# ZackAttack614/BlackBird

Measured on AMD Instinct MI355X. Metric: selfplay_games_per_sec, higher is better.
Workload: dtype f32 (float32 operands split exactly into 3 bf16 values, 6 bf16 MFMA products each, f32 accumulate)

## Files before the change

blackbird_amd/csrc/tree.hip.h:

```cpp
#pragma once
#include "games.hip.h"
#include "rng.hip.h"
#include "starts.h"
#include "stamps.hip.h"

#define NODE_EXPANDED 1
#define NODE_TERMINAL 2
#define NODE_CACHED 4
#define LEAF_RECORDED 0x40000000
#define CHILD_NONE (-1)
#define CHILD_TERM_BIT 0x40000000

template <class G>
struct alignas(128) DenseNode {
    int32_t flags;
    uint32_t legal_mask;
    int32_t all;
    int32_t serial;
    double sq;
    double pad0;
    int32_t N[G::S];
    float Q[G::S];
    int32_t child[G::S];
    alignas(128) double cP[G::S];
    float W[G::S];
    typename G::State st;
};

struct ExampleHdr {
    uint32_t game_id;
    uint16_t ply;
    uint8_t player;
    int8_t z;
    uint32_t total;
    uint32_t n_children;
};

#define BB_SLOTS_TREE(B, Q, R)                                                                     \
    B(int32_t, root, 1) B(int32_t, root_N, 1) B(int32_t, n_nodes, 1) B(int32_t, ply, 1) B(int32_t, sims_left, 1)           \
    B(int32_t, pend_leaf, 1) B(int32_t, pend_expand, 1) B(int32_t, path_len, 1)                                            \
    B(int32_t, game_lid, 1)                                             \
    B(int32_t, sim_serial, 1) B(float, root_W, 1)                                                                          \
    B(int8_t, root_pp, 1)                                   \
    B(uint32_t, path, MP)                                                                \
        \
    R(int32_t, path_N, MP) R(int32_t, path_all, MP)       \
    R(float, path_W, MP)                                                               \
    Q(int32_t, leaf_flags, 1)
#define BB_SLOTS_ANC(X)                                                                                 \
       \
    X(uint32_t, anc, ANC)                                                                                                   \
    X(int32_t, anc_len, 1) X(int32_t, top_N, 1)
#define BB_SLOTS_MAILBOX(B, Q)                                                 \
    B(uint32_t, leaf_game_id, 1) B(int32_t, leaf_serial, 1) B(float, eval_value, 1) Q(float, eval_policy, PS)              \
    B(uint64_t, evals, 1)                                                              \
    B(uint64_t, ctr, 8)
#define BB_SLOTS_OUT(X)                                                       \
    X(int32_t, out_action, 1) X(int32_t, out_root_plays, 1) X(int32_t, out_child_plays, S)                                 \
    X(float, out_root_winrate, 1) X(float, out_child_value, S)
#define BB_SLOTS_RESUME(X) X(int32_t, resume_cur, 1) X(int32_t, resume_depth, 1)
#define BB_SLOTS_POST(X) X(int, post_slot, 1)
#define BB_ROW_NONE(...)
#define BB_SLOT_ARRAYS(X) BB_SLOTS_TREE(X, X, X) BB_SLOTS_ANC(X) BB_SLOTS_MAILBOX(X, X) BB_SLOTS_OUT(X) BB_SLOTS_RESUME(X) BB_SLOTS_POST(X)
#define BB_SLOT_SHADOWED(X) BB_SLOTS_TREE(X, BB_ROW_NONE, BB_ROW_NONE) BB_SLOTS_MAILBOX(X, BB_ROW_NONE)
#define BB_SLOT_POINTER(T, f, per) T *f;
#define BB_SHADOW_MEMBER(T, f, per) T f[GW * (per)];
#define BB_SHADOW_LOAD(o, f, per) for (int i = threadIdx.x; i < n * (per); i += nthreads) f[i] = o.f[(size_t)g0 * (per) + i];
#define BB_SHADOW_STORE(o, f, per) for (int i = threadIdx.x; i < n * (per); i += nthreads) o.f[(size_t)g0 * (per) + i] = f[i];

struct TreeDev {
    int n_slots, node_cap, sims_per_move, max_plies, kind, max_depth, evaluator, priors_ones;
    int salt_per_game, max_games;
    int gpw;
    double c_puct;
    uint64_t seed, salt;
    uint32_t first_game_id;
    BB_SLOTS_TREE(BB_SLOT_POINTER, BB_SLOT_POINTER, BB_SLOT_POINTER)
    int track_anc;
    BB_SLOTS_ANC(BB_SLOT_POINTER)
    void *leaf_state;
    BB_SLOTS_MAILBOX(BB_SLOT_POINTER, BB_SLOT_POINTER)
    void *nodes;
    int n_games_target;
    double temp;
    uint8_t *examples;
    int32_t *game_hdr;
    int example_bytes;
    BB_SLOTS_OUT(BB_SLOT_POINTER)
    const double *in_u;
    BB_SLOTS_RESUME(BB_SLOT_POINTER)
    int *post_count;
    BB_SLOTS_POST(BB_SLOT_POINTER)
    int level_budget;
    int slot_offset;
    int lid_stride;
    int pool_g0;
    int *visit_pool;
    float noise_alpha;
    void *eval_cache;
    int eval_cache_log2;
    unsigned long long *eval_cache_ctr;
    unsigned long long *stamps;
    const void *starts;
    int n_starts;
    double temp_late;
    int temp_plies;
};

template <int STEP>
__device__ __forceinline__ int dpp_step_i(int v) {
    if (STEP == 0) return __builtin_amdgcn_update_dpp(v, v, 0xB1, 0xf, 0xf, false);
    if (STEP == 1) return __builtin_amdgcn_update_dpp(v, v, 0x4E, 0xf, 0xf, false);
    if (STEP == 2) return __builtin_amdgcn_update_dpp(v, v, 0x141, 0xf, 0xf, false);
    return __builtin_amdgcn_update_dpp(v, v, 0x140, 0xf, 0xf, false);
}
template <int STEP>
__device__ __forceinline__ double dpp_step_d(double v) {
    long long b = __double_as_longlong(v);
    int lo = dpp_step_i<STEP>((int)(b & 0xffffffffll)), hi = dpp_step_i<STEP>((int)(b >> 32));
    return __longlong_as_double(((long long)hi << 32) | (unsigned int)lo);
}

template <int S>
__device__ __forceinline__ int grp_sum_i(int v) {
    v += dpp_step_i<0>(v);
    v += dpp_step_i<1>(v);
    v += dpp_step_i<2>(v);
    if (S == 16) v += dpp_step_i<3>(v);
    return v;
}

template <int A, int S>
__device__ __forceinline__ double grp_np_sum(double x) {
    double a[A];
#pragma unroll
    for (int k = 0; k < A; k++) a[k] = __shfl(x, k, S);
    if (A < 8) {
        double res = 0.;
#pragma unroll
        for (int k = 0; k < A; k++) res += a[k];
        return res;
    } else {
        double r[8];
#pragma unroll
        for (int j = 0; j < 8; j++) r[j] = a[j];
        int i = 8;
        for (; i < A - (A % 8); i += 8)
            for (int j = 0; j < 8; j++) r[j] += a[i + j];
        double res = ((r[0] + r[1]) + (r[2] + r[3])) + ((r[4] + r[5]) + (r[6] + r[7]));
        for (; i < A; i++) res += a[i];
        return res;
    }
}

template <int S, int STEP>
__device__ __forceinline__ void argmax_step(double &u, int &idx, int &payload) {
    double ou = dpp_step_d<STEP>(u);
    int oi = dpp_step_i<STEP>(idx), op = dpp_step_i<STEP>(payload);
    if (ou > u || (ou == u && oi < idx)) {
        u = ou;
        idx = oi;
        payload = op;
    }
}
template <int S>
__device__ __forceinline__ int grp_argmax(double u, int idx, int &payload) {
    (void)idx;
    double m = u;
    m = __builtin_fmax(m, dpp_step_d<0>(m));
    m = __builtin_fmax(m, dpp_step_d<1>(m));
    m = __builtin_fmax(m, dpp_step_d<2>(m));
    if (S == 16) m = __builtin_fmax(m, dpp_step_d<3>(m));
    const unsigned long long eq = __ballot(u == m);
    const int l64 = (int)__lane_id();
    const unsigned grp = (unsigned)(eq >> (l64 & ~(S - 1))) & ((1u << S) - 1u);
    const int win = __ffs(grp) - 1;
    payload = __shfl(payload, win, S);
    return win;
}

__device__ __forceinline__ double puct_score(double q, double cPi, double sq, int Ni, bool legal) {
    double u = q + __ddiv_rn(cPi * sq, 1.0 + (double)Ni);
    return legal ? u : -1.0;
}
#ifndef BB_PUCT_FILTER
#define BB_PUCT_FILTER 1
#endif
template <int S>
__device__ __forceinline__ int grp_argmax_puct(float qf, double cPi, double sq, int Ni, bool legal, int &payload) {
#if BB_PUCT_FILTER
    const float num = (float)(cPi * sq);
    const float uf = legal ? __builtin_fmaf(num, __builtin_amdgcn_rcpf((float)(Ni + 1)), qf) : -1.0f;
    float mf = uf;
    mf = __builtin_fmaxf(mf, __int_as_float(dpp_step_i<0>(__float_as_int(mf))));
    mf = __builtin_fmaxf(mf, __int_as_float(dpp_step_i<1>(__float_as_int(mf))));
    mf = __builtin_fmaxf(mf, __int_as_float(dpp_step_i<2>(__float_as_int(mf))));
    if (S == 16) mf = __builtin_fmaxf(mf, __int_as_float(dpp_step_i<3>(__float_as_int(mf))));
    const bool mine = uf >= mf - mf * 0x1p-18f && uf >= 0.0f;
    const unsigned long long cand = __ballot(mine);
    const int l64 = (int)__lane_id();
    const unsigned grp = (unsigned)(cand >> (l64 & ~(S - 1))) & ((1u << S) - 1u);
    if (__ballot((grp & (grp - 1u)) != 0u || grp == 0u) == 0ull) {
        const int win = __ffs(grp) - 1;
        int p = mine ? payload : 0;
        p |= dpp_step_i<0>(p);
        p |= dpp_step_i<1>(p);
        p |= dpp_step_i<2>(p);
        if (S == 16) p |= dpp_step_i<3>(p);
        payload = p;
        return win;
    }
#endif
    return grp_argmax<S>(puct_score((double)qf, cPi, sq, Ni, legal), 0, payload);
}
__device__ __forceinline__ double child_q(const TreeDev &d, float Qi, float Wi, int Ni) {
    if (d.evaluator != 2) return (double)Qi;
    return Ni > 0 ? (double)Wi / (double)Ni : 0.0;
}

__device__ __forceinline__ uint32_t path_word(int node, int player, int a) {
    return ((uint32_t)node << 6) | ((uint32_t)player << 4) | (uint32_t)a;
}
#define ANC_BROKEN (-1)

template <class G, bool REC = false>
__device__ __forceinline__ void backup_path(const TreeDev &d, int g, int lane, DenseNode<G> *pool, int plen, float v01,
                                            int prev) {
    constexpr int S = G::S;
    const float vflip = 1.0f - v01;
    const size_t p0 = (size_t)g * G::MAXPATH;
    auto edge = [&](uint32_t e, int k) __attribute__((always_inline)) {
        const int a = e & 15, pl = (e >> 4) & 3;
        DenseNode<G> *pn = pool + (e >> 6);
        int n, all;
        float w;
        if constexpr (REC) { n = d.path_N[p0 + k]; all = d.path_all[p0 + k]; w = d.path_W[p0 + k]; }
        else { n = pn->N[a]; all = pn->all; w = pn->W[a]; }
        n += 1;
        all += 1;
        w += (pl == prev) ? v01 : vflip;
        pn->N[a] = n;
        pn->W[a] = w;
        pn->Q[a] = __fdiv_rn(w, (float)n);
        pn->all = all;
        pn->sq = __dsqrt_rn(1.0 + (double)all);
    };
    for (int k = lane; k < plen; k += S) edge(d.path[p0 + k], k);
    if constexpr (!REC) {
        if (d.track_anc) {
            const uint32_t *anc = d.anc + (size_t)g * (d.max_plies + 2);
            const int na = d.anc_len[g];
            for (int k = lane; k < na; k += S) edge(anc[k], 0);
            if (lane == 0) d.top_N[g] += 1;
        }
    }
    if (lane == 0) {
        d.root_N[g] += 1;
        int pp = d.root_pp[g];
        if (pp) d.root_W[g] += (pp == prev) ? v01 : vflip;
    }
}

template <class G, bool REC = false>
__device__ __forceinline__ void phase_apply(const TreeDev &d, int g, int lane) {
    using Node = DenseNode<G>;
    constexpr int S = G::S, A = G::A;
    const int leaf = d.pend_leaf[g];
    if (leaf < 0) return;
    int lf = 0;
    if constexpr (REC) lf = d.leaf_flags[g] & ~LEAF_RECORDED;
    Node *pool = (Node *)d.nodes + (size_t)(g + d.pool_g0) * d.node_cap;
    Node *node = pool + leaf;
    auto add_flag = [&](int bit) __attribute__((always_inline)) {
        if constexpr (REC) node->flags = lf | bit;
        else node->flags |= bit;
    };
    const typename G::State st = ((const typename G::State *)d.leaf_state)[g];
    const float v = d.eval_value[g];
    const int expand_rec = REC ? d.pend_expand[g] : 0;
    auto expand = [&]() __attribute__((always_inline)) { return REC ? expand_rec : d.pend_expand[g]; };
    if (expand()) {
        const uint32_t mask = G::legal_mask(st);
        double x = 0.0;
        if (lane < A) x = (double)d.eval_policy[(size_t)g * S + lane] * (double)((mask >> lane) & 1u);
        const double tot = grp_np_sum<A, S>(x);
        node->N[lane] = 0;
        node->Q[lane] = 0.f;
        node->W[lane] = 0.f;
        node->child[lane] = CHILD_NONE;
        node->cP[lane] = (lane < A) ? d.c_puct * __ddiv_rn(x, tot) : 0.0;
        if (lane == 0) {
            add_flag(NODE_EXPANDED);
            node->legal_mask = mask;
            node->all = 0;
            node->sq = 1.0;
        }
    }
    const int player = gs_player(st), prev = gs_prev(st);
    const bool f32_eval = REC || d.evaluator != 2;
    float v01 = v;
    if (f32_eval) {
        v01 = (v + 1.0f) * 0.5f;
        if (player != prev) v01 = 1.0f - v01;
    }
    if (f32_eval && !expand() && ((REC ? lf : node->flags) & NODE_TERMINAL) && lane == 0) {
        node->pad0 = (double)v01;
        add_flag(NODE_CACHED);
    }
    backup_path<G, REC>(d, g, lane, pool, d.path_len[g], v01, prev);
    if (lane == 0) d.pend_leaf[g] = -1;
}

template <class G>
__device__ __forceinline__ int create_child(const TreeDev &d, int g, DenseNode<G> *pool, DenseNode<G> *parent,
                                            const typename G::State &pst, int a, int lane, int &nn,
                                            typename G::State &st2, bool &terminal, int *flags_out = nullptr) {
    int idx = nn;
    st2 = pst;
    G::apply(st2, a);
    int w = G::winner(st2, a);
    terminal = w >= 0;
    if (idx >= d.node_cap) return CHILD_NONE;
    int word = idx | (terminal ? CHILD_TERM_BIT : 0);
    nn = idx + 1;
    const int cflags = (terminal ? (NODE_TERMINAL | ((w + 1) << 8)) : 0) | (gs_player(st2) << 4);
    if (flags_out) *flags_out = cflags;
    if (lane == 0) {
        DenseNode<G> *c = pool + idx;
        c->st = st2;
        c->flags = cflags;
        c->legal_mask = 0;
        c->all = 0;
        c->serial = idx;
        parent->child[a] = word;
        d.n_nodes[g] = idx + 1;
        d.ctr[(size_t)g * 8 + 2] += 1;
    }
    return word;
}

template <class G>
__device__ __forceinline__ uint32_t expand_ones(const TreeDev &d, DenseNode<G> *node, const typename G::State &st,
                                                int lane, double &cPi) {
    uint32_t mask = G::legal_mask(st);
    cPi = (lane < G::A && ((mask >> lane) & 1u)) ? d.c_puct * 1.0 : 0.0;
    node->N[lane] = 0;
    node->Q[lane] = 0.f;
    node->W[lane] = 0.f;
    node->child[lane] = CHILD_NONE;
    node->cP[lane] = cPi;
    if (lane == 0) {
        node->flags |= NODE_EXPANDED;
        node->legal_mask = mask;
        node->all = 0;
        node->sq = 1.0;
    }
    return mask;
}

template <class G>
__device__ __forceinline__ void post_leaf(const TreeDev &d, int g, int cur, const typename G::State &st, int flags_word, int expand,
                                          int depth) {
    ((typename G::State *)d.leaf_state)[g] = st;
    d.leaf_game_id[g] = d.first_game_id + (uint32_t)d.game_lid[g];
    d.leaf_serial[g] = cur;
    d.pend_leaf[g] = cur;
    if (d.leaf_flags) d.leaf_flags[g] = flags_word;
    d.pend_expand[g] = expand;
    d.path_len[g] = depth;
    d.sim_serial[g] += 1;
    d.evals[g] += 1;
}

template <class G>
__device__ void phase_select(const TreeDev &d, int g, int lane) {
    using Node = DenseNode<G>;
    constexpr int S = G::S, A = G::A;
    if (d.game_lid[g] < 0 || d.sims_left[g] <= 0) return;
    Node *pool = (Node *)d.nodes + (size_t)(g + d.pool_g0) * d.node_cap;
    uint32_t *path = d.path + (size_t)g * G::MAXPATH;
    int cur = d.root[g];
    int nn = d.n_nodes[g];
    int depth = 0, expand = 0, overflow = 0, term_leaf = 0;
    const bool inline_expand = d.priors_ones != 0;
    const bool fixed = d.kind == 1, rollout = d.evaluator == 2;
    typename G::State st;
    int flags = 0;
    bool have = false;
    IF_STAMPS(long long acc_load = 0, acc_iter = 0;)
    for (int it = 0;; it++) {
        IF_STAMPS(long long ts0 = clock64(); acc_iter++;)
        Node *node = pool + cur;
        typename G::State st_l = node->st;
        int flags_l = node->flags;
        uint32_t mask = node->legal_mask;
        double sq = node->sq;
        int Ni = node->N[lane];
        float Qi = node->Q[lane];
        float Wi = rollout ? node->W[lane] : 0.f;
        double cPi = node->cP[lane];
        int ci = node->child[lane];
        asm volatile("" ::"v"(flags_l), "v"(mask), "v"(sq), "v"(Ni), "v"(Qi), "v"(cPi), "v"(ci));
        IF_STAMPS(acc_load += clock64() - ts0;)
        if (!have) {
            st = st_l;
            flags = flags_l;
        }
        have = false;
        if (fixed && it >= d.max_depth) break;
        if (!(flags & NODE_EXPANDED)) {
            if (flags & NODE_TERMINAL) { term_leaf = 1; break; }
            if (!inline_expand) { expand = 1; break; }
            mask = expand_ones<G>(d, node, st, lane, cPi);
            if (!fixed) break;
            Ni = 0;
            Qi = 0.f;
            Wi = 0.f;
            sq = 1.0;
            ci = CHILD_NONE;
        }
        if (mask == 0) break;
        double u = puct_score(child_q(d, Qi, Wi, Ni), cPi, sq, Ni, lane < A && ((mask >> lane) & 1u));
        int child = ci;
        int a = grp_argmax<S>(u, lane, child);
        if (depth >= G::MAXPATH) { overflow = 1; break; }
        if (child == CHILD_NONE) {
            typename G::State st2;
            bool terminal;
            child = create_child<G>(d, g, pool, node, st, a, lane, nn, st2, terminal);
            if (child == CHILD_NONE) { overflow = 1; break; }
            if (lane == 0) path[depth] = path_word(cur, (flags >> 4) & 3, a);
            st = st2;
            flags = (terminal ? NODE_TERMINAL : 0) | (gs_player(st2) << 4);
            have = true;
        } else {
            if (lane == 0) path[depth] = path_word(cur, (flags >> 4) & 3, a);
        }
        depth++;
        cur = child & ~CHILD_TERM_BIT;
    }
    if (lane == 0) {
        IF_STAMPS(stamp_add(d.stamps, TS_ROW_LOAD, acc_load); stamp_add(d.stamps, TS_ITERATIONS, acc_iter); stamp_add(d.stamps, TS_DESCENTS, 1);)
        post_leaf<G>(d, g, cur, st, 0, expand, depth);
        d.sims_left[g] -= 1;
        uint64_t *c = d.ctr + (size_t)g * 8;
        c[0] += 1;
        c[1] += (uint64_t)depth;
        c[3] += (uint64_t)term_leaf;
        c[6] += (uint64_t)overflow;
    }
}

template <class G>
__global__ void __launch_bounds__(256) k_tree_step(TreeDev d) {
    constexpr int S = G::S;
    int t = blockIdx.x * blockDim.x + threadIdx.x;
    int wv = t >> 6, l64 = t & 63;
    if (l64 >= d.gpw * S) return;
    int g = wv * d.gpw + l64 / S, lane = l64 % S;
    if (g >= d.n_slots) return;
    const long long t0 = stamp_clock();
    phase_apply<G>(d, g, lane);
    const long long t1 = stamp_clock();
    __threadfence_block();
    const long long t2 = stamp_clock();
    phase_select<G>(d, g, lane);
    const long long t3 = stamp_clock();
    if ((threadIdx.x & 63) == 0) {
        stamp_add(d.stamps, TS_APPLY, t1 - t0);
        stamp_add(d.stamps, TS_FENCE, t2 - t1);
        stamp_add(d.stamps, TS_SELECT, t3 - t2);
        stamp_add(d.stamps, TS_WAVES, 1);
    }
}

template <class G>
__global__ void __launch_bounds__(256) k_tree_apply(TreeDev d) {
    constexpr int S = G::S;
    int t = blockIdx.x * blockDim.x + threadIdx.x;
    int g = t / S, lane = t % S;
    if (g >= d.n_slots) return;
    phase_apply<G>(d, g, lane);
}

template <class G>
__device__ __forceinline__ int choose_move(const TreeDev &d, int g, int lane, double temp, double u, int &total, int &Ni_out,
                           float &Wi_out) {
    using Node = DenseNode<G>;
    constexpr int S = G::S, A = G::A;
    Node *pool = (Node *)d.nodes + (size_t)(g + d.pool_g0) * d.node_cap;
    Node *node = pool + d.root[g];
    if (!(node->flags & NODE_EXPANDED)) {
        total = 0;
        Ni_out = 0;
        Wi_out = 0.f;
        return -3;
    }
    uint32_t mask = node->legal_mask;
    bool legal = lane < A && ((mask >> lane) & 1u);
    int Ni = legal ? node->N[lane] : 0;
    float Wi = legal ? node->W[lane] : 0.f;
    Ni_out = Ni;
    Wi_out = Wi;
    int all = grp_sum_i<S>(Ni);
    total = all;
    if (temp == 0.0) {
        double uu = puct_score(child_q(d, node->Q[lane], Wi, Ni), node->cP[lane], node->sq, Ni, legal);
        int dummy = 0;
        return grp_argmax<S>(uu, lane, dummy);
    }
    double it = 1.0 / temp;
    double w = (it == 1.0) ? (double)Ni : pow((double)Ni, it);
    double ws[A];
#pragma unroll
    for (int k = 0; k < A; k++) ws[k] = __shfl(w, k, S);
    double allp = 0.0;
#pragma unroll
    for (int k = 0; k < A; k++) allp += ws[k];
    if (!(allp > 0.0 && allp < INFINITY)) return -4;
    double last = 0.0;
#pragma unroll
    for (int k = 0; k < A; k++) last += __ddiv_rn(ws[k], allp);
    double run = 0.0;
    int act = A - 1;
    bool found = false;
#pragma unroll
    for (int k = 0; k < A; k++) {
        run += __ddiv_rn(ws[k], allp);
        if (!found && __ddiv_rn(run, last) > u) {
            act = k;
            found = true;
        }
    }
    return act;
}

template <class G>
__global__ void __launch_bounds__(256) k_sample(TreeDev d, double temp) {
    constexpr int S = G::S;
    int t = blockIdx.x * blockDim.x + threadIdx.x;
    int g = t / S, lane = t % S;
    if (g >= d.n_slots) return;
    if (d.game_lid[g] < 0) {
        if (lane == 0 && d.out_action) d.out_action[g] = -3;
        return;
    }
    double u = d.in_u ? d.in_u[g] : bb_u53(d.seed, d.first_game_id + (uint32_t)d.game_lid[g], (uint32_t)d.ply[g]);
    int total, Ni;
    float Wi;
    int act = choose_move<G>(d, g, lane, temp, u, total, Ni, Wi);
    if (d.out_child_plays) d.out_child_plays[(size_t)g * S + lane] = Ni;
    if (d.out_child_value) d.out_child_value[(size_t)g * S + lane] = Wi;
    if (lane == 0) {
        if (d.out_action) d.out_action[g] = act;
        if (d.out_root_plays) d.out_root_plays[g] = d.root_N[g];
        if (d.out_root_winrate) {
            int n = d.root_N[g];
            float w = d.root_W[g];
            d.out_root_winrate[g] = n > 0 ? ((d.evaluator == 2) ? (float)((double)w / (double)n) : __fdiv_rn(w, (float)n)) : 0.f;
        }
    }
}

template <class G, bool CHAIN = true>
__device__ __forceinline__ void advance_root(const TreeDev &d, int g, int lane, int a, typename G::State &new_st) {
    using Node = DenseNode<G>;
    Node *pool = (Node *)d.nodes + (size_t)(g + d.pool_g0) * d.node_cap;
    Node *node = pool + d.root[g];
    typename G::State st = node->st;
    if (!(node->flags & NODE_EXPANDED)) {
        new_st = st;
        G::apply(new_st, a);
        if (lane == 0) {
            Node *r = pool;
            r->st = new_st;
            r->flags = gs_player(new_st) << 4;
            r->serial = 0;
            d.n_nodes[g] = 1;
            d.root[g] = 0;
            d.root_N[g] = 0;
            d.root_W[g] = 0.f;
            d.root_pp[g] = 0;
            if (d.track_anc) {
                d.anc_len[g] = 0;
                d.top_N[g] = 0;
            }
        }
        return;
    }
    int child = node->child[a];
    int cn = node->N[a];
    float cw = node->W[a];
    if (child == CHILD_NONE) {
        bool terminal;
        int nn = d.n_nodes[g];
        child = create_child<G>(d, g, pool, node, st, a, lane, nn, new_st, terminal);
        if (child == CHILD_NONE) {
            child = 0;
            cn = 0;
            cw = 0.f;
            if (lane == 0) {
                pool->st = new_st;
                pool->flags = gs_player(new_st) << 4;
                d.n_nodes[g] = 1;
                d.ctr[(size_t)g * 8 + 6] += 1;
            }
        }
    } else {
        new_st = pool[child & ~CHILD_TERM_BIT].st;
    }
    if (lane == 0) {
        if (d.track_anc) {
            if (child == 0 && cn == 0 && d.n_nodes[g] == 1) {
                d.anc_len[g] = 0;
                d.top_N[g] = 0;
            } else if constexpr (!CHAIN) {
                if (d.anc_len[g] < d.max_plies + 2) {
                    d.anc[(size_t)g * (d.max_plies + 2) + d.anc_len[g]] = path_word(d.root[g], gs_player(st), a);
                    d.anc_len[g] += 1;
                }
            } else {
                const int na = d.anc_len[g], cap = d.max_plies + 2;
                if (na >= 0 && na < cap) {
                    d.anc[(size_t)g * cap + na] = path_word(d.root[g], gs_player(st), a);
                    d.anc_len[g] = na + 1;
                } else {
                    d.anc_len[g] = ANC_BROKEN;
                }
            }
        }
        d.root[g] = child & ~CHILD_TERM_BIT;
        d.root_N[g] = cn;
        d.root_W[g] = cw;
        d.root_pp[g] = (int8_t)gs_player(st);
    }
}

template <class G>
__global__ void __launch_bounds__(256) k_reset_roots(TreeDev d) {
    int g = blockIdx.x * blockDim.x + threadIdx.x;
    if (g >= d.n_slots || !d.track_anc || d.game_lid[g] < 0 || d.anc_len[g] <= 0) return;
    {
        const int na = d.anc_len[g];
        const bool parked = d.resume_cur[g] >= 0, posted = d.pend_leaf[g] >= 0;
        const int plen = parked ? d.resume_depth[g] : d.path_len[g];
        if (parked || posted) {
            if (plen + na <= G::MAXPATH) {
                uint32_t *path = d.path + (size_t)g * G::MAXPATH;
                const uint32_t *anc = d.anc + (size_t)g * (d.max_plies + 2);
                for (int k = plen - 1; k >= 0; k--) path[k + na] = path[k];
                for (int k = 0; k < na; k++) path[k] = anc[k];
                if (parked) d.resume_depth[g] = plen + na;
                else d.path_len[g] = plen + na;
            } else {
                d.ctr[(size_t)g * 8 + 6] += 1;
            }
        }
    }
    d.root[g] = (int)(d.anc[(size_t)g * (d.max_plies + 2)] >> 6);
    d.root_N[g] = d.top_N[g];
    d.root_W[g] = 0.f;
    d.root_pp[g] = 0;
    d.anc_len[g] = 0;
}

template <class G>
__global__ void __launch_bounds__(64) k_node_view(TreeDev d, int g, int node, int32_t *child_out, int32_t *plays_out, float *value_out,
                                                   typename G::State *state_out, int32_t *info_out) {
    using Node = DenseNode<G>;
    const int lane = threadIdx.x;
    if (lane >= G::S) return;
    Node *pool = (Node *)d.nodes + (size_t)(g + d.pool_g0) * d.node_cap;
    if (node < 0) node = d.root[g];
    const Node *n = pool + node;
    const bool exp = (n->flags & NODE_EXPANDED) != 0;
    child_out[lane] = exp ? n->child[lane] : CHILD_NONE;
    plays_out[lane] = exp ? n->N[lane] : 0;
    value_out[lane] = exp ? n->W[lane] : 0.f;
    if (lane == 0) {
        *state_out = n->st;
        info_out[0] = n->flags;
        info_out[1] = (int32_t)(exp ? n->legal_mask : 0u);
        info_out[2] = node;
    }
}

template <class G>
__global__ void __launch_bounds__(256) k_move_roots(TreeDev d, const int32_t *actions) {
    constexpr int S = G::S;
    int t = blockIdx.x * blockDim.x + threadIdx.x;
    int g = t / S, lane = t % S;
    if (g >= d.n_slots) return;
    int a = actions[g];
    if (a < 0 || a >= G::A || d.game_lid[g] < 0) return;
    typename G::State ns;
    advance_root<G>(d, g, lane, a, ns);
    if (lane == 0) d.ply[g] += 1;
}

template <class G>
__device__ __forceinline__ void reset_slot(const TreeDev &d, int g, int lid, const typename G::State &st) {
    using Node = DenseNode<G>;
    Node *pool = (Node *)d.nodes + (size_t)(g + d.pool_g0) * d.node_cap;
    pool->st = st;
    pool->flags = gs_player(st) << 4;
    pool->legal_mask = 0;
    pool->all = 0;
    pool->serial = 0;
    d.n_nodes[g] = 1;
    d.root[g] = 0;
    d.root_N[g] = 0;
    d.root_W[g] = 0.f;
    d.root_pp[g] = 0;
    d.ply[g] = 0;
    d.pend_leaf[g] = -1;
    d.pend_expand[g] = 0;
    d.path_len[g] = 0;
    d.sim_serial[g] = 0;
    d.game_lid[g] = lid;
    if (d.leaf_flags) d.leaf_flags[g] = 0;
    if (d.track_anc) {
        d.anc_len[g] = 0;
        d.top_N[g] = 0;
    }
}

template <class G>
__global__ void __launch_bounds__(256) k_set_roots(TreeDev d, int n, const int32_t *slots,
                                                   const typename G::State *states, const uint32_t *game_ids) {
    int i = blockIdx.x * blockDim.x + threadIdx.x;
    if (i >= n) return;
    int g = slots ? slots[i] : i;
    if (g < 0 || g >= d.n_slots) return;
    reset_slot<G>(d, g, game_ids ? (int)game_ids[i] : g, states[i]);
    d.sims_left[g] = 0;
}

__global__ void __launch_bounds__(256) k_add_sims(TreeDev d, int sims, const uint8_t *mask = nullptr) {
    int g = blockIdx.x * blockDim.x + threadIdx.x;
    if (g >= d.n_slots) return;
    if (d.game_lid[g] >= 0 && (!mask || mask[g])) d.sims_left[g] = sims;
}

template <class G>
__global__ void __launch_bounds__(256) k_get_roots(TreeDev d, typename G::State *out) {
    int g = blockIdx.x * blockDim.x + threadIdx.x;
    if (g >= d.n_slots) return;
    out[g] = ((DenseNode<G> *)d.nodes + (size_t)(g + d.pool_g0) * d.node_cap + d.root[g])->st;
}

template <class G>
__device__ __forceinline__ typename G::State start_state(const TreeDev &d, int lid) {
    const typename G::State *t = (const typename G::State *)d.starts;
    if (t && lid >= 0) return t[lid % d.n_starts];
    return G::initial();
}

template <class G>
__global__ void __launch_bounds__(256) k_check_starts(int n, const typename G::State *states, uint8_t *verdict) {
    int i = blockIdx.x * blockDim.x + threadIdx.x;
    if (i >= n) return;
    const typename G::State st = states[i];
    int v = BB_START_OK;
    if (G::winner(st, -1) >= 0) v = BB_START_FINISHED;
    else if (G::legal_mask(st) == 0) v = BB_START_NO_MOVE;
    verdict[i] = (uint8_t)v;
}

template <class G>
__global__ void __launch_bounds__(256) k_selfplay_begin(TreeDev d) {
    int g = blockIdx.x * blockDim.x + threadIdx.x;
    if (g >= d.n_slots) return;
    if (g + d.slot_offset < d.n_games_target) {
        reset_slot<G>(d, g, g + d.slot_offset, start_state<G>(d, g + d.slot_offset));
        d.sims_left[g] = d.sims_per_move;
    } else {
        reset_slot<G>(d, g, -1, start_state<G>(d, -1));
        d.sims_left[g] = 0;
    }
}

template <class G>
__device__ __forceinline__ uint8_t *example_ptr(const TreeDev &d, int lid, int ply) {
    return d.examples + ((size_t)lid * (d.max_plies + 1) + ply) * d.example_bytes;
}

template <class G>
__device__ __forceinline__ void write_example(const TreeDev &d, int lid, int ply, const typename G::State &st, int lane, int Ni,
                              int total, uint32_t gid) {
    uint8_t *p = example_ptr<G>(d, lid, ply);
    if (lane == 0) {
        ExampleHdr h;
        h.game_id = gid;
        h.ply = (uint16_t)ply;
        h.player = (uint8_t)gs_player(st);
        h.z = 0;
        h.total = (uint32_t)total;
        h.n_children = G::A;
        *(ExampleHdr *)p = h;
        *(typename G::State *)(p + sizeof(ExampleHdr)) = st;
    }
    ((uint32_t *)(p + sizeof(ExampleHdr) + sizeof(typename G::State)))[lane] = (uint32_t)Ni;
}

template <class G, bool CHAIN = true>
__device__ __forceinline__ void selfplay_move_body(const TreeDev &d, int g, int lane) {
    using Node = DenseNode<G>;
    constexpr int S = G::S;
    int lid = d.game_lid[g];
    if (lid < 0) return;
    Node *pool = (Node *)d.nodes + (size_t)(g + d.pool_g0) * d.node_cap;
    typename G::State st = pool[d.root[g]].st;
    uint32_t gid = d.first_game_id + (uint32_t)lid;
    int ply = d.ply[g];
    double u = bb_u53(d.seed, gid, (uint32_t)ply);
    int total, Ni;
    float Wi;
    int act = choose_move<G>(d, g, lane, ply < d.temp_plies ? d.temp : d.temp_late, u, total, Ni, Wi);
    if (act < 0) {
        if (lane == 0) {
            d.game_lid[g] = -1;
            d.ctr[(size_t)g * 8 + 6] += 1;
        }
        return;
    }
    write_example<G>(d, lid, ply, st, lane, Ni, total, gid);
    typename G::State ns;
    advance_root<G, CHAIN>(d, g, lane, act, ns);
    __threadfence_block();
    ply += 1;
    int w = G::winner(ns, -1);
    bool over = w >= 0 || ply >= d.max_plies;
    if (!over) {
        if (lane == 0) {
            d.ply[g] = ply;
            d.sims_left[g] = d.sims_per_move;
            d.ctr[(size_t)g * 8 + 5] += 1;
        }
        return;
    }
    write_example<G>(d, lid, ply, ns, lane, 0, 0, gid);
    __threadfence_block();
    for (int k = lane; k <= ply; k += S) {
        ExampleHdr *h = (ExampleHdr *)example_ptr<G>(d, lid, k);
        h->z = (w <= 0) ? 0 : (h->player == w ? 1 : -1);
    }
    __threadfence();
    if (lane == 0) {
        int32_t *gh = d.game_hdr + (size_t)lid * 4;
        gh[0] = ply + 1;
        gh[1] = w;
        gh[2] = ply;
        __threadfence();
        gh[3] = 1;
        uint64_t *c = d.ctr + (size_t)g * 8;
        c[4] += 1;
        c[5] += 1;
        c[7] += (uint64_t)(ply + 1);
        int next = lid + d.lid_stride;
        if (next < d.n_games_target) {
            reset_slot<G>(d, g, next, start_state<G>(d, next));
            d.sims_left[g] = d.sims_per_move;
        } else {
            d.game_lid[g] = -1;
            d.sims_left[g] = 0;
        }
    }
}

template <class G>
__global__ void __launch_bounds__(256) k_selfplay_move(TreeDev d) {
    constexpr int S = G::S;
    int t = blockIdx.x * blockDim.x + threadIdx.x;
    int g = t / S, lane = t % S;
    if (g >= d.n_slots) return;
    phase_apply<G>(d, g, lane);
    __threadfence_block();
    selfplay_move_body<G>(d, g, lane);
}

struct NoPostHook {
    __device__ __forceinline__ void operator()(int, int) const {}
};
template <class G, bool REC = false, class OnPost = NoPostHook>
__device__ bool async_game(const TreeDev &d, int g, int lane, OnPost on_post = OnPost(), LevelStamps *light_out = nullptr) {
    using Node = DenseNode<G>;
    constexpr int S = G::S, A = G::A;
    if (d.game_lid[g] < 0) return false;
    Node *pool = (Node *)d.nodes + (size_t)(g + d.pool_g0) * d.node_cap;
    LevelStamps light;
    if (d.pend_leaf[g] >= 0) {
        if (REC && (d.leaf_flags[g] & LEAF_RECORDED)) phase_apply<G, true>(d, g, lane);
        else phase_apply<G>(d, g, lane);
        if (lane == 0) d.sims_left[g] -= 1;
        __threadfence_block();
    }
    int budget = d.level_budget;
    uint32_t *path = d.path + (size_t)g * G::MAXPATH;
    int sims_done = 0, depth_sum = 0, term_hits = 0;
    bool posted = false;
    for (;;) {
        if (d.sims_left[g] <= 0) {
            selfplay_move_body<G, !REC>(d, g, lane);
            __threadfence_block();
            if (d.game_lid[g] < 0) break;
        }
        int cur = d.resume_cur[g], depth = 0;
        if (cur >= 0) depth = d.resume_depth[g];
        else cur = d.root[g];
        int nn = d.n_nodes[g];
        typename G::State st;
        int flags = 0;
        enum { F_PARKED = 2, F_LEAF = 4, F_TERM = 8, F_EXPAND = 16, F_OVERFLOW = 32 };
        int fl = 0;
        IF_STAMPS_LIGHT(int lt_e = (int)clock64();)
        for (;;) {
            if (budget <= 0) { fl |= F_PARKED; break; }
            budget--;
            IF_STAMPS_LIGHT(light.levels++; int lt_a = (int)clock64();)
            Node *node = pool + cur;
            typename G::State st_l = node->st;
            int flags_l = node->flags;
            uint32_t mask = node->legal_mask;
            double sq = node->sq;
            int Ni = node->N[lane];
            float Qi = node->Q[lane];
            double cPi = node->cP[lane];
            int ci = node->child[lane];
            double cached = node->pad0;
            float Wi = 0.f;
            int all_l = 0;
            if (REC) {
                Wi = node->W[lane];
                all_l = node->all;
            }
            asm volatile("" ::"v"(flags_l), "v"(mask), "v"(sq), "v"(Ni), "v"(Qi), "v"(cPi), "v"(ci));
            IF_STAMPS_LIGHT(int lt_b = (int)clock64(); light.row_load += lt_b - lt_a;)
            st = st_l;
            flags = flags_l;
            if (!(flags & NODE_EXPANDED)) {
                fl |= F_LEAF;
                if (flags & NODE_TERMINAL) {
                    fl |= F_TERM;
                    if (flags & NODE_CACHED) {
                        float v01 = (float)cached;
                        __threadfence_block();
                        backup_path<G, REC>(d, g, lane, pool, depth, v01, gs_prev(st));
                        if (lane == 0) d.sims_left[g] -= 1;
                        __threadfence_block();
                        sims_done++;
                        depth_sum += depth;
                        term_hits++;
                        fl &= ~F_LEAF;
                    }
                } else {
                    fl |= F_EXPAND;
                }
                break;
            }
            static_assert(G::MAXPATH >= G::H * G::W + 2, "a descent places at most H*W stones");
            int child = ci;
            int a = grp_argmax_puct<S>(Qi, cPi, sq, Ni, lane < A && ((mask >> lane) & 1u), child);
            IF_STAMPS_LIGHT(asm volatile("" ::"v"(a), "v"(child)); light.puct += (int)clock64() - lt_b;)
            if (lane == 0) path[depth] = path_word(cur, (flags >> 4) & 3, a);
            if (REC) {
                if (lane == 0) d.path_all[(size_t)g * G::MAXPATH + depth] = all_l;
                if (lane == a) {
                    d.path_N[(size_t)g * G::MAXPATH + depth] = Ni;
                    d.path_W[(size_t)g * G::MAXPATH + depth] = Wi;
                }
            }
            if (child == CHILD_NONE) {
                typename G::State st2;
                bool terminal;
                child = create_child<G>(d, g, pool, node, st, a, lane, nn, st2, terminal, &flags);
                if (child == CHILD_NONE) { fl |= F_OVERFLOW | F_LEAF; break; }
                st = st2;
                depth++;
                cur = child & ~CHILD_TERM_BIT;
                fl |= F_LEAF | (terminal ? F_TERM : F_EXPAND);
                break;
            }
            depth++;
            cur = child & ~CHILD_TERM_BIT;
        }
        IF_STAMPS_LIGHT(light.loop += (int)clock64() - lt_e;)
        if (lane == 0) {
            d.resume_cur[g] = (fl & F_PARKED) ? cur : -1;
            d.resume_depth[g] = (fl & F_PARKED) ? depth : 0;
        }
        if (fl & F_PARKED) break;
        if (!(fl & F_LEAF)) {
            if (lane == 0) d.sim_serial[g] += 1;
            continue;
        }
        if (lane == 0) {
            post_leaf<G>(d, g, cur, st, REC ? (flags | LEAF_RECORDED) : 0, (fl & F_EXPAND) ? 1 : 0, depth);
            d.ctr[(size_t)g * 8 + 6] += (uint64_t)((fl & F_OVERFLOW) ? 1 : 0);
        }
        on_post(g, lane);
        sims_done++;
        depth_sum += depth;
        term_hits += (fl & F_TERM) ? 1 : 0;
        posted = true;
        break;
    }
    if (light_out) *light_out = light;
    if (lane == 0 && sims_done) {
        uint64_t *c = d.ctr + (size_t)g * 8;
        c[0] += (uint64_t)sims_done;
        c[1] += (uint64_t)depth_sum;
        c[3] += (uint64_t)term_hits;
    }
    return posted;
}

template <class G>
__global__ void __launch_bounds__(256) k_tree_async(TreeDev d, int round) {
    constexpr int S = G::S;
    int t = blockIdx.x * blockDim.x + threadIdx.x;
    int wv = t >> 6, l64 = t & 63;
    int g = wv * d.gpw + l64 / S, lane = l64 % S;
    bool live = l64 < d.gpw * S && g < d.n_slots;
    LevelStamps light;
    bool posted = live ? async_game<G>(d, g, lane, NoPostHook(), &light) : false;
    level_stamps_flush(d.stamps, light, live && lane == 0, l64);
    unsigned long long m = __ballot(posted && lane == 0);
    if (t == 0) d.post_count[(round + 2) & 3] = 0;
    if (m) {
        int leader = __ffsll((long long)m) - 1;
        int base = 0;
        if (l64 == leader) base = atomicAdd(&d.post_count[round & 3], __popcll(m));
        base = __shfl(base, leader, 64);
        if (posted && lane == 0) d.post_slot[base + __popcll(m & ((1ull << l64) - 1ull))] = g;
    }
}
```

Measured before the change: 9307.

## Cache terminal values in parent rows and reorder node layout for hot fields

```diff
diff --git a/blackbird_amd/csrc/node_row.h b/blackbird_amd/csrc/node_row.h
--- /dev/null
+++ b/blackbird_amd/csrc/node_row.h
@@ -0,0 +1,23 @@
+#pragma once
+#include <cstddef>
+#include <cstdint>
+
+#define CHILD_NONE (-1)
+#define CHILD_TERM_BIT 0x40000000
+#define CHILD_TVAL_BIT 0x20000000
+#define CHILD_INDEX_MASK 0x1FFFFFFF
+
+template <int S, int A, class State>
+struct alignas(128) DenseRow {
+    int32_t N[S];
+    float Q[S];
+    int32_t child[S];
+    double sq;
+    int32_t flags;
+    uint32_t legal_mask;
+    int32_t all;
+    float tv[A];
+    double cP[S];
+    float W[S];
+    State st;
+};
diff --git a/blackbird_amd/csrc/tree.hip.h b/blackbird_amd/csrc/tree.hip.h
--- a/blackbird_amd/csrc/tree.hip.h
+++ b/blackbird_amd/csrc/tree.hip.h
@@ -3,29 +3,17 @@
 #include "rng.hip.h"
 #include "starts.h"
 #include "stamps.hip.h"
+#include "node_row.h"
 
 #define NODE_EXPANDED 1
 #define NODE_TERMINAL 2
 #define NODE_CACHED 4
 #define LEAF_RECORDED 0x40000000
-#define CHILD_NONE (-1)
-#define CHILD_TERM_BIT 0x40000000
-
-template <class G>
-struct alignas(128) DenseNode {
-    int32_t flags;
-    uint32_t legal_mask;
-    int32_t all;
-    int32_t serial;
-    double sq;
-    double pad0;
-    int32_t N[G::S];
-    float Q[G::S];
-    int32_t child[G::S];
-    alignas(128) double cP[G::S];
-    float W[G::S];
-    typename G::State st;
-};
+
+template <class G>
+using DenseNode = DenseRow<G::S, G::A, typename G::State>;
+static_assert(sizeof(DenseNode<Connect4>) == 256 && alignof(DenseNode<Connect4>) == 128, "a Connect4 row is two 128-byte lines");
+static_assert(sizeof(DenseNode<TicTacToe>) == 512 && alignof(DenseNode<TicTacToe>) == 128, "a TicTacToe row is four");
 
 struct ExampleHdr {
     uint32_t game_id;
@@ -304,8 +292,15 @@
         if (player != prev) v01 = 1.0f - v01;
     }
     if (f32_eval && !expand() && ((REC ? lf : node->flags) & NODE_TERMINAL) && lane == 0) {
-        node->pad0 = (double)v01;
+        node->tv[0] = v01;
         add_flag(NODE_CACHED);
+        const int plen = d.path_len[g];
+        if (plen > 0) {
+            const uint32_t e = d.path[(size_t)g * G::MAXPATH + plen - 1];
+            Node *pn = pool + (e >> 6);
+            pn->tv[e & 15] = v01;
+            pn->child[e & 15] = leaf | CHILD_TERM_BIT | CHILD_TVAL_BIT;
+        }
     }
     backup_path<G, REC>(d, g, lane, pool, d.path_len[g], v01, prev);
     if (lane == 0) d.pend_leaf[g] = -1;
@@ -331,7 +326,6 @@
         c->flags = cflags;
         c->legal_mask = 0;
         c->all = 0;
-        c->serial = idx;
         parent->child[a] = word;
         d.n_nodes[g] = idx + 1;
         d.ctr[(size_t)g * 8 + 2] += 1;
@@ -437,7 +431,7 @@
             if (lane == 0) path[depth] = path_word(cur, (flags >> 4) & 3, a);
         }
         depth++;
-        cur = child & ~CHILD_TERM_BIT;
+        cur = child & CHILD_INDEX_MASK;
     }
     if (lane == 0) {
         IF_STAMPS(stamp_add(d.stamps, TS_ROW_LOAD, acc_load); stamp_add(d.stamps, TS_ITERATIONS, acc_iter); stamp_add(d.stamps, TS_DESCENTS, 1);)
@@ -575,7 +569,6 @@
             Node *r = pool;
             r->st = new_st;
             r->flags = gs_player(new_st) << 4;
-            r->serial = 0;
             d.n_nodes[g] = 1;
             d.root[g] = 0;
             d.root_N[g] = 0;
@@ -607,7 +600,7 @@
             }
         }
     } else {
-        new_st = pool[child & ~CHILD_TERM_BIT].st;
+        new_st = pool[child & CHILD_INDEX_MASK].st;
     }
     if (lane == 0) {
         if (d.track_anc) {
@@ -629,7 +622,7 @@
                 }
             }
         }
-        d.root[g] = child & ~CHILD_TERM_BIT;
+        d.root[g] = child & CHILD_INDEX_MASK;
         d.root_N[g] = cn;
         d.root_W[g] = cw;
         d.root_pp[g] = (int8_t)gs_player(st);
@@ -674,7 +667,8 @@
     if (node < 0) node = d.root[g];
     const Node *n = pool + node;
     const bool exp = (n->flags & NODE_EXPANDED) != 0;
-    child_out[lane] = exp ? n->child[lane] : CHILD_NONE;
+    const int cw = exp ? n->child[lane] : CHILD_NONE;
+    child_out[lane] = cw == CHILD_NONE ? cw : cw & ~CHILD_TVAL_BIT;
     plays_out[lane] = exp ? n->N[lane] : 0;
     value_out[lane] = exp ? n->W[lane] : 0.f;
     if (lane == 0) {
@@ -706,7 +700,6 @@
     pool->flags = gs_player(st) << 4;
     pool->legal_mask = 0;
     pool->all = 0;
-    pool->serial = 0;
     d.n_nodes[g] = 1;
     d.root[g] = 0;
     d.root_N[g] = 0;
@@ -911,15 +904,16 @@
         int nn = d.n_nodes[g];
         typename G::State st;
         int flags = 0;
-        enum { F_PARKED = 2, F_LEAF = 4, F_TERM = 8, F_EXPAND = 16, F_OVERFLOW = 32 };
+        enum { F_PARKED = 2, F_LEAF = 4, F_TERM = 8, F_EXPAND = 16, F_OVERFLOW = 32, F_CACHED = 64 };
         int fl = 0;
+        float v01 = 0.f;
+        int prev = 0;
         IF_STAMPS_LIGHT(int lt_e = (int)clock64();)
         for (;;) {
             if (budget <= 0) { fl |= F_PARKED; break; }
             budget--;
             IF_STAMPS_LIGHT(light.levels++; int lt_a = (int)clock64();)
             Node *node = pool + cur;
-            typename G::State st_l = node->st;
             int flags_l = node->flags;
             uint32_t mask = node->legal_mask;
             double sq = node->sq;
@@ -927,34 +921,24 @@
             float Qi = node->Q[lane];
             double cPi = node->cP[lane];
             int ci = node->child[lane];
-            double cached = node->pad0;
+            float tvi = node->tv[lane < A ? lane : 0];
             float Wi = 0.f;
             int all_l = 0;
             if (REC) {
                 Wi = node->W[lane];
                 all_l = node->all;
             }
-            asm volatile("" ::"v"(flags_l), "v"(mask), "v"(sq), "v"(Ni), "v"(Qi), "v"(cPi), "v"(ci));
+            asm volatile("" ::"v"(flags_l), "v"(mask), "v"(sq), "v"(Ni), "v"(Qi), "v"(cPi), "v"(ci), "v"(tvi));
             IF_STAMPS_LIGHT(int lt_b = (int)clock64(); light.row_load += lt_b - lt_a;)
-            st = st_l;
             flags = flags_l;
             if (!(flags & NODE_EXPANDED)) {
-                fl |= F_LEAF;
-                if (flags & NODE_TERMINAL) {
-                    fl |= F_TERM;
-                    if (flags & NODE_CACHED) {
-                        float v01 = (float)cached;
-                        __threadfence_block();
-                        backup_path<G, REC>(d, g, lane, pool, depth, v01, gs_prev(st));
-                        if (lane == 0) d.sims_left[g] -= 1;
-                        __threadfence_block();
-                        sims_done++;
-                        depth_sum += depth;
-                        term_hits++;
-                        fl &= ~F_LEAF;
-                    }
+                st = node->st;
+                if ((flags & (NODE_TERMINAL | NODE_CACHED)) == (NODE_TERMINAL | NODE_CACHED)) {
+                    fl |= F_TERM | F_CACHED;
+                    v01 = node->tv[0];
+                    prev = gs_prev(st);
                 } else {
-                    fl |= F_EXPAND;
+                    fl |= F_LEAF | ((flags & NODE_TERMINAL) ? F_TERM : F_EXPAND);
                 }
                 break;
             }
@@ -973,16 +957,24 @@
             if (child == CHILD_NONE) {
                 typename G::State st2;
                 bool terminal;
+                st = node->st;
                 child = create_child<G>(d, g, pool, node, st, a, lane, nn, st2, terminal, &flags);
                 if (child == CHILD_NONE) { fl |= F_OVERFLOW | F_LEAF; break; }
                 st = st2;
                 depth++;
-                cur = child & ~CHILD_TERM_BIT;
+                cur = child & CHILD_INDEX_MASK;
                 fl |= F_LEAF | (terminal ? F_TERM : F_EXPAND);
                 break;
             }
             depth++;
-            cur = child & ~CHILD_TERM_BIT;
+            if (child & CHILD_TVAL_BIT) {
+                fl |= F_TERM | F_CACHED;
+                budget--;
+                v01 = __shfl(tvi, a, S);
+                prev = (flags >> 4) & 3;
+                break;
+            }
+            cur = child & CHILD_INDEX_MASK;
         }
         IF_STAMPS_LIGHT(light.loop += (int)clock64() - lt_e;)
         if (lane == 0) {
@@ -990,8 +982,17 @@
             d.resume_depth[g] = (fl & F_PARKED) ? depth : 0;
         }
         if (fl & F_PARKED) break;
-        if (!(fl & F_LEAF)) {
-            if (lane == 0) d.sim_serial[g] += 1;
+        if (fl & F_CACHED) {
+            __threadfence_block();
+            backup_path<G, REC>(d, g, lane, pool, depth, v01, prev);
+            if (lane == 0) {
+                d.sims_left[g] -= 1;
+                d.sim_serial[g] += 1;
+            }
+            __threadfence_block();
+            sims_done++;
+            depth_sum += depth;
+            term_hits++;
             continue;
         }
         if (lane == 0) {
```

Result: no change. 9219 (median of 2 runs) (-1.0%).
